# leok7v/sqz

Hardware: AMD Instinct MI355X
Metric: encode MB/s + decode MB/s, 32KB window, batched blocks, 1/2/4/8 MI355X (higher is better)
Workload: dtype u8; 1 GPU; 4096 x 262144 B Zipf(s=1) byte blocks, window 2^15, one independent stream per block (BASELINE.json configs[2]); total_blocks=4096, blocks_per_gpu=4096, block_bytes=262144, win_bits=15, parallelism=1 rank; the N>1 runs shard this same batch (strong scaling), finder=index, device=AMD Radeon Graphics (gfx950:sramecc+:xnack-)

## Files before the change

sqz_amd/csrc/decode.hip:

```cpp
#define SQZ_CHANGED_INLINING __forceinline__
#define SQZ_INSERT_INLINING __forceinline__
#define SQZ_LUT_INLINING __forceinline__
#include "sqz_tree.h"
#include "sqz_kernels.h"

namespace sqzk {

constexpr int kStageDw = 128;

struct DecodeLuts {
    uint16_t lit[1 << 8];
    uint16_t pos[1 << 6];
};

struct DecodeLds {
    TreeLds    tree;
    DecodeLuts luts;
    uint32_t   stage[kStageDw];
};

using LitTree = LitTreeT<false, false>;
using PosTree = PosTreeT<false, false>;

template <class T>
// ... 253 lines not shown
#endif
            ST_SEC(0)
            const int hop = ok ? (int)used : 128;
            uint64_t starts = 0;
            uint32_t s = 0;
            do {
                set_bit64(starts, s);
                s += (uint32_t)__builtin_amdgcn_readlane(hop, (int)s);
            } while (s < (uint32_t)kWave);
            if (s >= 128u) {
                stop = true;
                const int last = 63 - __builtin_clzll(starts);
                starts &= ~(1ull << last);
                s = (uint32_t)last;
            }
            base += s;
            if ((starts >> lane) & 1ull) {
                const int at = m + (int)__builtin_amdgcn_mbcnt_hi((uint32_t)(starts >> 32),
                                   __builtin_amdgcn_mbcnt_lo((uint32_t)starts, 0u));
                slot[at] = word | ((used - 1u) << 25);
            }
            m += __builtin_popcountll(starts);
            ST_SEC(1)
        }
        m = m < kWave ? m : kWave;
        ST_SEC(1)
        lds_fence();
        uint32_t word_v = 0, used_v = 0, slot_v = 0;
        if (lane < m) { slot_v = slot[lane]; word_v = slot_v & 0x81FFFFFFu; used_v = ((slot_v >> 25) & 63u) + 1u; }
        const bool is_match = (word_v & kTokMatch) != 0;
        const uint32_t tlen_v = lane < m ? (is_match ? ((word_v >> 16) & 0x1FFu) : 1u) : 0u;
        uint32_t scan = (used_v << 16) | tlen_v;
        scan = wave_scan(scan);
        const uint64_t out_before = i + (uint64_t)((scan & 0xFFFFu) - tlen_v);
        const bool invalid = lane < m &&
            (out_before >= bytes ||
             (is_match && ((uint64_t)(word_v & 0x7FFFu) > out_before + (kHist ? history : 0u) || (uint64_t)tlen_v > bytes - out_before)));
        const uint64_t inv = __ballot(invalid);
        if (inv != 0) { const int f = __builtin_ctzll(inv); if (f < m) { m = f; stop = true; } }
        int a_v = -1, b_v = -1;
        if (lane < m) {
            if (is_match) {
                a_v = kSymLen0 + len_code((int)tlen_v).code;
                b_v = kPosBase + pos_code((int)(word_v & 0x7FFFu)).code;
            } else {
                a_v = (int)word_v;
            }
        }
        uint32_t ca, cb;
        int wa, wb;
        int done = 0;
        ST_SEC(2)
        lds_fence();
        if (m > 0) { done = bump_batch<false>(&lds.tree, nullptr, lit, pos, lane, m, a_v, b_v, ca, wa, cb, wb); }
        ST_SEC(3)
        uint64_t resume = bit0;
        if (done > 0) {
            if (lane < done) { tok[ntok + (uint32_t)lane] = word_v; }
            const uint32_t af = (uint32_t)__builtin_amdgcn_readlane((int)scan, done - 1);
            ntok += (uint32_t)done;
            i += (uint64_t)(af & 0xFFFFu);
            resume = bit0 + (uint64_t)(af >> 16);
        }
#ifdef SQZ_STATS
        st_steps++; st_m += (uint32_t)m; st_done += (uint32_t)done;
#ifdef SQZ_STATS_SERIES
        if (lane == 0 && b == 1) { printf("S %d %d %d %d\n", want, m, done, (int)stop); }
#endif
        st_hist[done == 0 ? 0 : done < 8 ? 1 : done < 24 ? 2 : done < 64 ? 3 : 4]++;
#endif
        ST_SEC(4)
        if (i < bytes && (stop || done < m)) {
            const bool may_keep = done + 1 < m;
            if (may_keep && lane == 0) {
                lds.tree.pend[LitTree::kChgSlot] = 0x7FFFFFFFu; lds.tree.pend[LitTree::kChgSlot + 1] = 0u;
                lds.tree.pend[PosTree::kChgSlot] = 0x7FFFFFFFu; lds.tree.pend[PosTree::kChgSlot + 1] = 0u;
            }
            lds_fence();
            if (done < m) {
                const int sa = __builtin_amdgcn_readlane(a_v, done), sb = __builtin_amdgcn_readlane(b_v, done);
                const uint32_t w1 = (uint32_t)__builtin_amdgcn_readlane((int)word_v, done);
                const uint32_t u1 = (uint32_t)__builtin_amdgcn_readlane((int)used_v, done);
                const uint32_t l1 = (uint32_t)__builtin_amdgcn_readlane((int)tlen_v, done);
                { const Chain c = lit.chain_up(sa, lane); (void)lit.bump_wave(sa, c, lane); }
                if (sb >= 0) { const Chain c = pos.chain_up(sb, lane); (void)pos.bump_wave(sb, c, lane); }
                if (lit.fault | pos.fault) { err = kE2BIG; }
                else {
                    if (lane == 0) { tok[ntok] = w1; }
                    ntok++;
                    i += (uint64_t)l1;
                    r.seek(resume + (uint64_t)u1);
                }
            } else {
                r.seek(resume);
                decode_one();
            }
            lds_fence();
            const bool still = (lit.complete | pos.complete) == 0 && lit.depth < kFreezeDepth && pos.depth < kFreezeDepth &&
                               (lit.aux & pos.aux) != 0;
            if (may_keep && still && err == 0 && i < bytes) {
                const uint32_t la = lds.tree.pend[LitTree::kChgSlot], ha = lds.tree.pend[LitTree::kChgSlot + 1];
                const uint32_t lb = lds.tree.pend[PosTree::kChgSlot], hb = lds.tree.pend[PosTree::kChgSlot + 1];
                const bool cand = lane > done && lane < m;
                bool moved = false;
                if (cand) {
                    const uint32_t qa = r_pos(lds.tree.rng[a_v]);
                    moved = qa >= la && qa < ha;
// ... 382 lines not shown
                    if (fin >= (uint32_t)kWave) { stop = true; advance = (uint32_t)(kWave * v) + (fin - (uint32_t)kWave); }
                    else { entry = fin; advance = (uint32_t)(kWave * (v + 1)) + fin; }
                }
            }
            if (mine) {
                uint64_t starts = 0;
                uint32_t s1 = my_entry;
                while (s1 < (uint32_t)kWave) {
                    const uint32_t h = (uint32_t)__builtin_amdgcn_readlane(hop, (int)s1);
                    if (h >= 1024u) { break; }
                    set_bit64(starts, s1);
                    s1 += h;
                }
                if ((starts >> lane) & 1ull) { slot[my_base + (int)lanes_under(starts)] = word | ((used - 1u) << 25); }
            }
            base += advance;
            MW_SEC(3)
        }
        }
        MW_SEC(5)
        if (shared) { lds_barrier(); }
        if (wave != 0) { continue; }
        const int m_total = m;
        m = m < kWave ? m : kWave;
        lds_fence();
        uint32_t word_v = 0, used_v = 0, slot_v = 0;
        if (lane < m) { slot_v = slot[lane]; word_v = slot_v & 0x81FFFFFFu; used_v = ((slot_v >> 25) & 63u) + 1u; }
        const bool is_match = (word_v & kTokMatch) != 0;
        const uint32_t tlen_v = lane < m ? (is_match ? ((word_v >> 16) & 0x1FFu) : 1u) : 0u;
        uint32_t scan = (used_v << 16) | tlen_v;
        scan = wave_scan(scan);
        const uint64_t out_before = i + (uint64_t)((scan & 0xFFFFu) - tlen_v);
        const bool invalid = lane < m &&
            (out_before >= bytes ||
             (is_match && ((uint64_t)(word_v & 0x7FFFu) > out_before + (kHist ? history : 0u) || (uint64_t)tlen_v > bytes - out_before)));
        const uint64_t inv = __ballot(invalid);
        if (inv != 0) { const int f = __builtin_ctzll(inv); if (f < m) { m = f; stop = true; } }
        int a_v = -1, b_v = -1;
        if (lane < m) {
            if (is_match) {
                a_v = kSymLen0 + len_code((int)tlen_v).code;
                b_v = kPosBase + pos_code((int)(word_v & 0x7FFFu)).code;
            } else {
                a_v = (int)word_v;
            }
        }
        uint32_t ca, cb;
        int wa, wb;
        int done = 0;
        MW_SEC(6)
#ifdef SQZ_STATS
        mw_steps++;
#endif
        if (m > 0) { done = bump_batch<false>(&lds.tree, nullptr, lit, pos, lane, m, a_v, b_v, ca, wa, cb, wb); }
        MW_SEC(7)
#ifdef SQZ_STATS
        mw_done += (uint32_t)done;
#endif
        uint64_t resume = bit0;
        if (done > 0) {
            if (lane < done) { tok[ntok + (uint32_t)lane] = word_v; }
            const uint32_t af = (uint32_t)__builtin_amdgcn_readlane((int)scan, done - 1);
            ntok += (uint32_t)done;
            i += (uint64_t)(af & 0xFFFFu);
            resume = bit0 + (uint64_t)(af >> 16);
        }
        kept = 0; kept_bits = 0;
        int keep_from = done;
        if (i < bytes && (stop || done < m)) {
            const bool may_keep = done + 1 < m;
            if (may_keep && lane == 0) {
                lds.tree.pend[LitTree::kChgSlot] = 0x7FFFFFFFu; lds.tree.pend[LitTree::kChgSlot + 1] = 0u;
                lds.tree.pend[PosTree::kChgSlot] = 0x7FFFFFFFu; lds.tree.pend[PosTree::kChgSlot + 1] = 0u;
            }
            lds_fence();
            if (done < m) {
                const int sa = __builtin_amdgcn_readlane(a_v, done), sb = __builtin_amdgcn_readlane(b_v, done);
                const uint32_t w1 = (uint32_t)__builtin_amdgcn_readlane((int)word_v, done);
                const uint32_t u1 = (uint32_t)__builtin_amdgcn_readlane((int)used_v, done);
                const uint32_t l1 = (uint32_t)__builtin_amdgcn_readlane((int)tlen_v, done);
                { const Chain c = lit.chain_up(sa, lane); (void)lit.bump_wave(sa, c, lane); }
                if (sb >= 0) { const Chain c = pos.chain_up(sb, lane); (void)pos.bump_wave(sb, c, lane); }
                if (lit.fault | pos.fault) { err = kE2BIG; }
                else {
                    if (lane == 0) { tok[ntok] = w1; }
                    ntok++;
                    i += (uint64_t)l1;
                    r.seek(resume + (uint64_t)u1);
                }
            } else {
                r.seek(resume);
                decode_one();
            }
            lds_fence();
            const bool still = (lit.complete | pos.complete) == 0 && lit.depth < kFreezeDepth && pos.depth < kFreezeDepth &&
                               (lit.aux & pos.aux) != 0;
            if (may_keep && still && err == 0 && i < bytes) {
                const uint32_t la = lds.tree.pend[LitTree::kChgSlot], ha = lds.tree.pend[LitTree::kChgSlot + 1];
                const uint32_t lb = lds.tree.pend[PosTree::kChgSlot], hb = lds.tree.pend[PosTree::kChgSlot + 1];
                const bool cand = lane > done && lane < m;
                bool moved = false;
                if (cand) {
                    const uint32_t qa = r_pos(lds.tree.rng[a_v]);
                    moved = qa >= la && qa < ha;
                    if (is_match) { const uint32_t qb = r_pos(lds.tree.rng[b_v]); moved |= qb >= lb && qb < hb; }
                }
                const uint64_t behind = ~0ull << (done + 1);
// ... 220 lines not shown
```

sqz_amd/csrc/huffman_emit.hip:

```cpp
#define SQZ_SEC_TIMERS
#define SQZ_CHANGED_INLINING __forceinline__
#define SQZ_INSERT_INLINING __forceinline__
#include "sqz_tree.h"
#include "sqz_kernels.h"

namespace sqzk {

constexpr int kPendBits = 58;

struct EmitLds {
    TreeLds  tree;
    uint32_t code[kCodeSlots];
};


struct BitQueue {
    EmitLds* lds;
    uint8_t* out;
    uint64_t capacity;
    uint64_t bytes;
    uint64_t carry_v;
    int      carry;
    int      error;
    uint64_t pend_v;
    int      pend_n;

    __device__ __forceinline__ void store_words(int words, int lane) {
        if (error != 0 || words == 0) { return; }
        const uint64_t room = capacity - bytes;
        for (int k = lane; k < words; k += kWave) {
            const uint64_t w = lds->tree.P64[k];
            const uint64_t at = (uint64_t)k * 8;
            if (at + 8 <= room) {
                *reinterpret_cast<uint64_t*>(out + bytes + at) = __builtin_bswap64(w);
            } else {
                for (int j = 0; j < 8; j++) {
                    if (at + (uint64_t)j < room) { out[bytes + at + j] = (uint8_t)(w >> (56 - 8 * j)); }
                }
            }
        }
        if ((uint64_t)words * 8 <= room) { bytes += (uint64_t)words * 8; }
        else { bytes = capacity; error = kE2BIG; }
    }

    __device__ __forceinline__ void deposit(uint64_t v, uint32_t n, uint32_t o) {
        const uint32_t w = o >> 6, s = o & 63u;
        if (s + n <= 64) {
            atomicOr(reinterpret_cast<unsigned long long*>(&lds->tree.P64[w]),
                     (unsigned long long)v << (64 - s - n));
        } else {
            const uint32_t r = s + n - 64;
            atomicOr(reinterpret_cast<unsigned long long*>(&lds->tree.P64[w]),
                     (unsigned long long)(v >> r));
            atomicOr(reinterpret_cast<unsigned long long*>(&lds->tree.P64[w + 1]),
                     (unsigned long long)v << (64 - r));
        }
    }

    __device__ __forceinline__ void pack_lanes(uint64_t v1, uint32_t n1, uint64_t v2, uint32_t n2, int lane) {
        for (int k = lane; k < kImageWords; k += kWave) { lds->tree.P64[k] = (k == 0) ? carry_v : 0ull; }
        lds_fence();
        const uint32_t incl = wave_scan(n1 + n2);
        const uint32_t head = (uint32_t)carry + (uint32_t)pend_n;
        const uint32_t total = (uint32_t)__builtin_amdgcn_readlane((int)incl, kWave - 1) + head;
        if (pend_n != 0 && lane == 0) { deposit(pend_v, (uint32_t)pend_n, (uint32_t)carry); }
        const uint32_t at = head + incl - (n1 + n2);
        if (n1 != 0) { deposit(v1, n1, at); }
        if (n2 != 0) { deposit(v2, n2, at + n1); }
        lds_fence();
        const int words = (int)(total >> 6);
        store_words(words, lane);
        carry_v = uni64(lds->tree.P64[words]);
        lds_fence();
        carry = (int)(total & 63u);
        pend_v = 0; pend_n = 0;
    }

    __device__ __forceinline__ void pack(int lane) {
        if (pend_n != 0) { pack_lanes(0ull, 0u, 0ull, 0u, lane); }
    }

    __device__ __forceinline__ void push32(uint32_t value, int width, int lane) {
        if (pend_n + width > kPendBits) { pack(lane); }
        const uint64_t bits = width >= 32 ? (uint64_t)value : (uint64_t)(value & ((1u << width) - 1u));
        pend_v = (pend_v << width) | bits;
        pend_n += width;
    }
    __device__ __forceinline__ void push(uint64_t value, int width, int lane) {
        if (width > 32) {
            push32((uint32_t)(value >> 32), width - 32, lane);
            push32((uint32_t)value, 32, lane);
        } else {
            push32((uint32_t)value, width, lane);
        }
    }
    __device__ __forceinline__ void push_lsb(uint32_t value, int width, int lane) {
        push32(__brev(value) >> (32 - width), width, lane);
    }

    __device__ __forceinline__ void flush(int lane) {
        pack(lane);
        if (carry > 0) {
            if (lane == 0) { lds->tree.P64[0] = carry_v; }
            lds_fence();
            store_words(1, lane);
            carry = 0; carry_v = 0;
        }
    }
};

__device__ __noinline__ uint64_t deep_code(const uint32_t* lnk, int leaf, int& width) {
    uint64_t code = 0;
    int n = 0, a = leaf;
    for (;;) {
        const uint32_t up = (uint32_t)__builtin_amdgcn_readfirstlane((int)l_up(lnk[a]));
        if (up == kNil || n >= 63) { break; }
        const uint32_t pw = (uint32_t)__builtin_amdgcn_readfirstlane((int)lnk[up]);
        code |= (uint64_t)(l_hi(pw) == (uint32_t)a ? 1 : 0) << n;
        a = (int)up;
        n++;
    }
    width = n;
    return code;
}

template <class T>
__device__ __forceinline__ void emit_coded(BitQueue& q, T& t, int s, int nyt, int raw_bits,
                                           int lane, int& err) {
    Chain c = t.chain_up(s, lane);
    const bool unseen = (c.levels == 0);
    if (unseen) { c = t.chain_up(nyt, lane); }
    const int leaf = unseen ? nyt : s;
    int width = c.levels;
    uint64_t deep = 0;
    if (width >= kMaxFastDepth) { deep = deep_code(t.lds->lnk, leaf, width); }
    uint64_t code = t.bump_wave(leaf, c, lane);
    if (c.levels >= kMaxFastDepth) { code = deep; }
    q.push(code, width, lane);
    if (unseen) {
        q.push_lsb((uint32_t)(s - T::kBase), raw_bits, lane);
        if (!t.insert_wave(s, lane)) { err = kE2BIG; }
    }
}

template <class LitTree, class PosTree>
__device__ __forceinline__ void emit_token(BitQueue& q, LitTree& lit, PosTree& pos, uint32_t t,
                                           int lane, int& err) {
    const bool is_match = (t & kTokMatch) != 0;
    Code lc = {0, 0, 0};
    int s_lit = (int)(t & 0xFFu);
    if (is_match) {
        lc = len_code((int)((t >> 16) & 0x1FFu));
        s_lit = kSymLen0 + lc.code;
    }
    emit_coded(q, lit, s_lit, kLitNyt, 9, lane, err);
    if (is_match) {
        if (lc.xbits > 0) { q.push_lsb((uint32_t)lc.extra, lc.xbits, lane); }
        const Code pc = pos_code((int)(t & 0x7FFFu));
        emit_coded(q, pos, kPosBase + pc.code, kPosBase + kPosNyt, 5, lane, err);
        if (pc.xbits > 0) { q.push_lsb((uint32_t)pc.extra, pc.xbits, lane); }
    }
    if (q.error != 0) { err = q.error; }
    if (lit.fault | pos.fault) { err = kE2BIG; }
}

__device__ __forceinline__ bool token_ok(uint32_t t) {
    if ((t & kTokMatch) == 0) { return t <= 0xFFu; }
    const uint32_t len = (t >> 16) & 0x7FFFu, dist = t & 0xFFFFu;
    return len >= (uint32_t)kLenMin && len <= (uint32_t)kLenMax && dist >= 1u && dist <= 0x7FFFu;
}

template <bool kStats>
__global__ __launch_bounds__(kWave, kStats ? 1 : 4)
void huffman_emit_kernel(const uint32_t* __restrict__ tokens,
                         const uint64_t* __restrict__ tok_off,
                         const uint32_t* __restrict__ tok_count,
                         uint8_t* __restrict__ out,
                         const uint64_t* __restrict__ out_off,
                         uint64_t* __restrict__ out_bytes,
                         int32_t* __restrict__ err_out,
                         uint32_t n_blocks,
                         uint64_t prefix_acc, int prefix_fill,
                         sqz_block_stats* __restrict__ stats_out) {
    __shared__ EmitLds lds;
    const int lane = threadIdx.x;
    const uint32_t b = blockIdx.x;
    if (b >= n_blocks) { return; }

    using LitTree = LitTreeT<true, kStats>;
    using PosTree = PosTreeT<true, kStats>;
    LitTree lit; PosTree pos;
    lit.lds = &lds.tree; lit.code = lds.code; lit.lut = nullptr;
    pos.lds = &lds.tree; pos.code = lds.code; pos.lut = nullptr;
    lit.init_all(lane);
    pos.init_all(lane);
    for (int k = lane; k < kCodeSlots; k += kWave) { lds.code[k] = 0; }
    __syncthreads();

    const uint32_t* tok = tokens + uni64(tok_off[b]);
    uint32_t count = (uint32_t)__builtin_amdgcn_readfirstlane((int)tok_count[b]);
    const bool too_many = (uint64_t)count > uni64(tok_off[b + 1]) - uni64(tok_off[b]);
    if (too_many) { count = 0; }

    BitQueue q;
    q.lds = &lds;
    const uint64_t o0 = uni64(out_off[b]), o1 = uni64(out_off[b + 1]);
    q.out = out + o0;
    q.capacity = o1 - o0;
    q.bytes = 0;
    q.pend_v = 0;
    q.pend_n = 0;
    q.carry = prefix_fill;
    q.carry_v = prefix_fill > 0 ? (prefix_acc << (64 - prefix_fill)) : 0ull;
    q.error = 0;
    int err = 0;

    if (too_many) { err = kEINVAL; }
    if (!lit.insert_wave(kLitNyt, lane)) { err = kEINVAL; }
    if (!pos.insert_wave(kPosBase + kPosNyt, lane)) { err = kEINVAL; }

    uint32_t cursor = 0;
    uint32_t lit_tokens = 0, match_bytes = 0;
    uint32_t win0 = (uint32_t)lane < count ? tok[lane] : 0u;
    uint32_t win1 = (uint32_t)lane + (uint32_t)kWave < count ? tok[kWave + lane] : 0u;
#ifdef SQZ_STATS
    uint64_t es[4] = {0, 0, 0, 0}, es_last = __builtin_readcyclecounter(), es_begin = es_last;
    uint32_t es_steps = 0, es_exact = 0;
#define ES(k) { const uint64_t n_ = __builtin_readcyclecounter(); es[k] += n_ - es_last; es_last = n_; }
#else
#define ES(k)
#endif
    const uint32_t quarter = (count >> 2) + 1;
    int prio_now = -1;
    int want = 16, avg4 = 32;
    uint32_t regain_at = 0;
    while (cursor < count && err == 0) {
        {
            const int qq = (int)(cursor / quarter);
            if (qq != prio_now) {
                prio_now = qq;
                if (qq == 0) { __builtin_amdgcn_s_setprio(3); }
                else if (qq == 1) { __builtin_amdgcn_s_setprio(2); }
                else if (qq == 2) { __builtin_amdgcn_s_setprio(1); }
                else { __builtin_amdgcn_s_setprio(0); }
            }
        }
        const uint32_t step_start = cursor;
        const bool valid = cursor + (uint32_t)lane < count;
        const uint32_t traw = win0;
        const bool wellformed = token_ok(traw);
        const uint32_t t = wellformed ? traw : 0u;
        const bool is_match = (t & kTokMatch) != 0;
        Code lc = {0, 0, 0}, pc = {0, 0, 0};
        int a = (int)(t & 0xFFu), bsym = -1;
        uint32_t tlen = 1;
        if (is_match) {
            tlen = (t >> 16) & 0x1FFu;
            lc = len_code((int)tlen);
            pc = pos_code((int)(t & 0x7FFFu));
            a = kSymLen0 + lc.code;
            bsym = kPosBase + pc.code;
        }
        const bool new_a = valid && l_up(lds.tree.lnk[a]) == kNil;
        const bool new_b = valid && is_match && l_up(lds.tree.lnk[bsym]) == kNil;
        const uint64_t unseen = __ballot(valid && (new_a || new_b || !wellformed));
        const uint64_t vmask = __ballot(valid);
        int m = unseen != 0 ? __builtin_ctzll(unseen) : __builtin_popcountll(vmask);
        m = m < want ? m : want;
        if (cursor > kBatchTokens && (lit.aux | pos.aux) != 0) {
            lit.give_up_aux(lane);
            pos.give_up_aux(lane);
        }
        if ((lit.aux & pos.aux) == 0 && cursor <= kBatchTokens && cursor >= regain_at) {
            regain_at = cursor + 512u;
            (void)lit.regain_aux(lane);
            (void)pos.regain_aux(lane);
        }
        const bool frozen = (lit.complete | pos.complete) != 0 || lit.depth >= kFreezeDepth || pos.depth >= kFreezeDepth ||
                            (lit.aux & pos.aux) == 0;
        uint32_t ca = 0, cb = 0;
        int wa = 0, wb = 0;
        const int offered = m;
        ES(0)
        if (m >= 1 && !frozen) { m = bump_batch<true>(&lds.tree, lds.code, lit, pos, lane, m, a, bsym, ca, wa, cb, wb); }
        else { m = 0; }
        ES(1)
        if (m >= 1) {
            uint64_t v1 = ca, v2 = 0;
            uint32_t n1 = (uint32_t)wa, n2 = 0;
            if (is_match) {
                v1 = (v1 << lc.xbits) | (uint64_t)(lc.xbits ? (__brev((uint32_t)lc.extra) >> (32 - lc.xbits)) : 0u);
                n1 += (uint32_t)lc.xbits;
                v2 = ((uint64_t)cb << pc.xbits) | (uint64_t)(pc.xbits ? (__brev((uint32_t)pc.extra) >> (32 - pc.xbits)) : 0u);
                n2 = (uint32_t)(wb + pc.xbits);
            }
            if (lane >= m) { n1 = 0; n2 = 0; }
            q.pack_lanes(v1, n1, v2, n2, lane);
            if (kStats) {
                const uint64_t mm = __ballot(lane < m && is_match);
                lit_tokens += (uint32_t)(m - __builtin_popcountll(mm));
                match_bytes += wave_sum((lane < m && is_match) ? tlen : 0u);
            }
            cursor += (uint32_t)m;
        }
        ES(2)
        if (m < offered || offered == 0 || frozen) {
            const uint32_t tx = (uint32_t)__builtin_amdgcn_readlane((int)traw, m);
            if (!token_ok(tx)) { err = kEINVAL; break; }
            emit_token(q, lit, pos, tx, lane, err);
            if (kStats) { if ((tx & kTokMatch) != 0) { match_bytes += (tx >> 16) & 0x1FFu; } else { lit_tokens += 1; } }
            cursor += 1;
#ifdef SQZ_STATS
            es_exact++;
#endif
        }
        ES(3)
#ifdef SQZ_EMU_DEBUG_BATCH
        if (lane == 0) {
            static unsigned dbg_steps = 0, dbg_offered = 0, dbg_applied = 0, dbg_exact = 0, dbg_next = 16384;
            dbg_steps++; dbg_offered += (unsigned)offered - g_dbg_cut; g_dbg_cut = 0; dbg_applied += (unsigned)m; dbg_exact += (m < offered || offered == 0 || frozen) ? 1u : 0u;
            if (cursor >= dbg_next || cursor >= count) {
                fprintf(stderr, "cursor %u: steps %u offered %u applied %u exact %u (want %d) depth %d/%d aux %d/%d\n", cursor, dbg_steps, dbg_offered, dbg_applied, dbg_exact, want,
                        lit.depth, pos.depth, lit.aux, pos.aux);
                dbg_steps = dbg_offered = dbg_applied = dbg_exact = 0; dbg_next = cursor + 16384;
            }
        }
#endif
#ifdef SQZ_STATS
        es_steps++;
#endif
        {
            avg4 += (int)(cursor - step_start) - (avg4 >> 2);
            want = ((avg4 * 3) >> 3) + 6;
            want = want < kWave ? want : kWave;
        }
        {
            const uint32_t adv = cursor - step_start;
            const int from = ((lane + (int)adv) & (kWave - 1)) * 4;
            const uint32_t s0 = (uint32_t)__builtin_amdgcn_ds_bpermute(from, (int)win0);
            const uint32_t s1 = (uint32_t)__builtin_amdgcn_ds_bpermute(from, (int)win1);
            win0 = (uint32_t)lane + adv < (uint32_t)kWave ? s0 : s1;
            const uint32_t t1 = cursor + (uint32_t)kWave + (uint32_t)lane;
            win1 = t1 < count ? tok[t1] : 0u;
        }
        if (q.error != 0) { err = q.error; }
        if (lit.fault | pos.fault) { err = kE2BIG; }
    }

#ifdef SQZ_STATS
    if (lane == 0 && b == 1) {
        printf("emit block 1: cycles %llu steps %u exact %u: prep %llu bump %llu pack %llu exact %llu\n",
               (unsigned long long)(es_last - es_begin), es_steps, es_exact, (unsigned long long)es[0],
               (unsigned long long)es[1], (unsigned long long)es[2], (unsigned long long)es[3]);
        for (int k = 0; k < 32; k++) { if (g_secn[k]) { printf("sec %d: %llu cycles / %u = %llu\n", k, g_sec[k], g_secn[k], g_sec[k] / g_secn[k]); } }
        printf("emit slow: lit insert %u/%llu changed %u/%llu; pos insert %u/%llu changed %u/%llu\n",
               lit.st_cnt[0], (unsigned long long)lit.st_cyc[0], lit.st_cnt[1], (unsigned long long)lit.st_cyc[1],
               pos.st_cnt[0], (unsigned long long)pos.st_cyc[0], pos.st_cnt[1], (unsigned long long)pos.st_cyc[1]);
    }
#endif
    if (err == 0) { q.flush(lane); err = q.error; }
    else { q.pack(lane); }
    if (lane == 0) {
        out_bytes[b] = q.bytes;
        err_out[b] = err;
        if (kStats && stats_out != nullptr) {
            sqz_block_stats* st = stats_out + b;
            st->lit_updates = lit.stats.updates; st->lit_swaps = lit.stats.swaps; st->lit_moves = lit.stats.moves;
            st->pos_updates = pos.stats.updates; st->pos_swaps = pos.stats.swaps; st->pos_moves = pos.stats.moves;
            st->literal_bytes = lit_tokens; st->backref_bytes = match_bytes;
            st->lit_depth = (uint32_t)lit.depth; st->pos_depth = (uint32_t)pos.depth;
            st->tokens = cursor; st->reserved = 0;
        }
    }
    if (kStats && stats_out != nullptr) {
        for (int k = lane; k < kLitLeaves; k += kWave) { stats_out[b].lit_freq[k] = lit.freq(k); }
        if (lane < kPosLeaves) { stats_out[b].pos_freq[lane] = pos.freq(kPosBase + lane); }
    }
}

using DbgLit = LitTreeT<true, true>;
using DbgPos = PosTreeT<true, true>;
template <class T>
__device__ __forceinline__ void debug_drive(T& t, DbgLit& lit, DbgPos& pos, EmitLds& lds, const int32_t* symbols,
                                            uint32_t count, int batch, int lane, bool is_pos, bool stop_early,
                                            uint32_t max_steps, uint32_t& consumed) {
    uint32_t k = 0;
    for (uint32_t step = 0; k < count && t.fault == 0 && (max_steps == 0 || step < max_steps); step++) {
        if (stop_early && t.aux == 0) { break; }
        int sym = -1;
        if (k + (uint32_t)lane < count) { sym = symbols[k + lane]; }
        const bool valid = sym >= 0 && sym < T::kLeaves && lane < batch;
        const int leaf = valid ? T::kBase + sym : T::kRoot;
        const uint64_t seen = __ballot(valid && l_up(lds.tree.lnk[leaf]) != kNil);
        int m = (~seen == 0ull) ? kWave : __builtin_ctzll(~seen);
        const bool frozen = t.complete != 0 || t.depth >= kFreezeDepth || t.aux == 0;
        uint32_t ca, cb; int wa, wb;
        if (m > 0 && !frozen) {
            m = is_pos ? bump_batch<true>(&lds.tree, lds.code, lit, pos, lane, m, -1, leaf, ca, wa, cb, wb)
                       : bump_batch<true>(&lds.tree, lds.code, lit, pos, lane, m, leaf, -1, ca, wa, cb, wb);
        } else { m = 0; }
        k += (uint32_t)m;
        if (k < count) {
            const int s = __builtin_amdgcn_readfirstlane(symbols[k]);
            if (s < 0 || s >= T::kLeaves) { break; }
            const int lf = T::kBase + s;
            const Chain c = t.chain_up(lf, lane);
            if (c.levels == 0) { (void)t.insert_wave(lf, lane); }
            else { (void)t.bump_wave(lf, c, lane); }
            k++;
        }
    }
    consumed = k;
}

__global__ __launch_bounds__(kWave, 4)
void tree_debug_kernel(const int32_t* __restrict__ symbols, uint32_t count, int which, int batch,
                       uint32_t* __restrict__ dump) {
    __shared__ EmitLds lds;
    const int lane = threadIdx.x;
    DbgLit lit; DbgPos pos;
    lit.lds = &lds.tree; lit.code = lds.code; lit.lut = nullptr;
    pos.lds = &lds.tree; pos.code = lds.code; pos.lut = nullptr;
    lit.init_all(lane);
    pos.init_all(lane);
    for (int k = lane; k < kCodeSlots; k += kWave) { lds.code[k] = 0; }
    __syncthreads();
    const bool stop_early = (batch & 0x100) != 0;
    batch &= 0xFF;
    if (batch < 1) { batch = 1; }
    if (batch > kWave) { batch = kWave; }
    const uint32_t max_steps = (uint32_t)which >> 8;
    which &= 1;
    uint32_t consumed = 0;
    if (which == 0) { debug_drive(lit, lit, pos, lds, symbols, count, batch, lane, false, stop_early, max_steps, consumed); }
    else { debug_drive(pos, lit, pos, lds, symbols, count, batch, lane, true, stop_early, max_steps, consumed); }
    lds_fence();
    const int base = which == 0 ? 0 : kPosBase, nodes = which == 0 ? kLitNodes : kPosNodes;
    const int leaves = which == 0 ? kLitLeaves : kPosLeaves, pos0 = which == 0 ? 0 : kPosPos0;
    if (lane == 0) {
        const TreeStats st = which == 0 ? lit.stats : pos.stats;
        dump[0] = (uint32_t)(which == 0 ? lit.next : pos.next);
        dump[1] = (uint32_t)(which == 0 ? lit.depth : pos.depth);
        dump[2] = (uint32_t)(which == 0 ? lit.complete : pos.complete);
        dump[3] = (uint32_t)(which == 0 ? lit.aux : pos.aux);
        dump[4] = (uint32_t)(which == 0 ? lit.fault : pos.fault) | (max_steps != 0 ? consumed << 8 : 0u);
        dump[5] = st.updates; dump[6] = st.swaps; dump[7] = st.moves;
    }
    for (int v = lane; v < nodes; v += kWave) {
        dump[8 + 4 * v + 0] = lds.tree.lnk[base + v];
        dump[8 + 4 * v + 1] = lds.tree.rng[base + v];
        dump[8 + 4 * v + 2] = lds.tree.cnt[base + v];
        dump[8 + 4 * v + 3] = v < leaves ? lds.code[pos0 + v] : 0u;
// ... 28 lines not shown
```

sqz_amd/csrc/sqz_tree.h:

```cpp
#pragma once

#include "sqz_device.h"

namespace sqzk {

constexpr uint32_t kNil = 0x3FFu;
constexpr int kLitLeaves = 288;
constexpr int kLitNodes  = kLitLeaves + 288;
constexpr int kPosLeaves = 32;
constexpr int kPosNodes  = 64;
constexpr int kPosBase   = kLitNodes;
constexpr int kAllNodes  = kLitNodes + kPosNodes;
constexpr int kPosPos0   = kLitLeaves;
constexpr int kPositions = kLitLeaves + kPosLeaves;
constexpr int kCodeSlots = kPositions;

constexpr uint32_t kCountMask = (1u << 24) - 1u;
constexpr int kDepthShift = 24;

#ifndef SQZ_AUX_DEPTH
#define SQZ_AUX_DEPTH 26
#endif
#ifndef SQZ_MAX_FAST_DEPTH
#define SQZ_MAX_FAST_DEPTH 60
#endif
#ifndef SQZ_FREEZE_DEPTH
#define SQZ_FREEZE_DEPTH 63
#endif
#ifndef SQZ_BATCH_TOKENS
#define SQZ_BATCH_TOKENS ((1u << 24) - 256u)
#endif
constexpr uint32_t kBatchTokens = SQZ_BATCH_TOKENS;
constexpr int kAuxDepth = SQZ_AUX_DEPTH;
constexpr int kMaxFastDepth = SQZ_MAX_FAST_DEPTH;
constexpr int kFreezeDepth = SQZ_FREEZE_DEPTH;
constexpr int kStack = 128;
constexpr int kTokenBits = 2 * (kAuxDepth - 1) + 18;
constexpr int kPackWords = (63 + 58 + kWave * kTokenBits + 63) / 64 + 1;
constexpr int kImageWords = kPackWords > kWave ? kPackWords : kWave;

#ifdef SQZ_EMU_DEBUG_BATCH
static unsigned g_dbg_cut;
#endif

#if defined(SQZ_STATS) && defined(SQZ_SEC_TIMERS)
__device__ unsigned long long g_sec[32];
__device__ unsigned int g_secn[32];
#define SEC_BEGIN uint64_t sec_t_ = __builtin_readcyclecounter();
#define SEC(k) { const uint64_t n_ = __builtin_readcyclecounter(); if (blockIdx.x == 1 && threadIdx.x == 0) { g_sec[k] += n_ - sec_t_; g_secn[k]++; } sec_t_ = n_; }
#define XSEC_BEGIN uint64_t xsec_t_ = __builtin_readcyclecounter();
#define XSEC(k) { const uint64_t n_ = __builtin_readcyclecounter(); if (blockIdx.x == 1 && threadIdx.x == 0) { g_sec[k] += n_ - xsec_t_; g_secn[k]++; } xsec_t_ = n_; }
#else
#define SEC_BEGIN
#define SEC(k)
#define XSEC_BEGIN
#define XSEC(k)
#endif

struct TreeLds {
    uint32_t lnk[kAllNodes];
    uint32_t rng[kAllNodes];
    uint32_t cnt[kAllNodes];
    uint32_t pend[kWave];
    uint16_t lvl[kStack];
    union { uint64_t P64[kImageWords]; uint32_t P32[2 * kImageWords]; uint8_t P8[8 * kImageWords]; };
};

struct TreeStats { uint32_t updates, swaps, moves; };

__device__ __forceinline__ void lds_fence() {
    __builtin_amdgcn_fence(__ATOMIC_SEQ_CST, "wavefront");
    asm volatile("" ::: "memory");
}

__device__ __forceinline__ uint32_t l_up(uint32_t w) { return w & 0x3FFu; }
__device__ __forceinline__ uint32_t l_lo(uint32_t w) { return (w >> 10) & 0x3FFu; }
__device__ __forceinline__ uint32_t l_hi(uint32_t w) { return (w >> 20) & 0x3FFu; }
__device__ __forceinline__ uint32_t mk_lnk(uint32_t up, uint32_t lo, uint32_t hi) { return up | (lo << 10) | (hi << 20); }
__device__ __forceinline__ uint32_t r_pos(uint32_t w) { return w & 0x1FFu; }
__device__ __forceinline__ uint32_t r_first(uint32_t w) { return w & 0x3FFu; }
__device__ __forceinline__ uint32_t r_last(uint32_t w) { return (w >> 10) & 0x3FFu; }
__device__ __forceinline__ uint32_t r_pa(uint32_t w) { return (w >> 20) & 0x3FFu; }
constexpr uint32_t kEndsMask = 0xFFFFFu;
constexpr uint32_t kNoPos = 0x1FFu;
__device__ __forceinline__ uint32_t c_f(uint32_t w) { return w & kCountMask; }
__device__ __forceinline__ uint32_t c_d(uint32_t w) { return (w >> kDepthShift) & 0x3Fu; }

__device__ __forceinline__ uint32_t wave_max(uint32_t v) {
    auto mx = [](uint32_t a, uint32_t b) { return a > b ? a : b; };
    v = mx(v, (uint32_t)__builtin_amdgcn_update_dpp(0, (int)v, 0x111 , 0xf, 0xf, false));
    v = mx(v, (uint32_t)__builtin_amdgcn_update_dpp(0, (int)v, 0x112 , 0xf, 0xf, false));
    v = mx(v, (uint32_t)__builtin_amdgcn_update_dpp(0, (int)v, 0x114 , 0xf, 0xf, false));
    v = mx(v, (uint32_t)__builtin_amdgcn_update_dpp(0, (int)v, 0x118 , 0xf, 0xf, false));
    v = mx(v, (uint32_t)__builtin_amdgcn_update_dpp(0, (int)v, 0x142 , 0xa, 0xf, false));
    v = mx(v, (uint32_t)__builtin_amdgcn_update_dpp(0, (int)v, 0x143 , 0xc, 0xf, false));
    return (uint32_t)__builtin_amdgcn_readlane((int)v, kWave - 1);
}

__device__ __forceinline__ uint32_t wave_sum(uint32_t v) {
    return (uint32_t)__builtin_amdgcn_readlane((int)wave_scan(v), kWave - 1);
}

struct Chain {
    int mine, par;
    int levels;
    bool holds;
    bool active;
    bool has_g;
};

#ifndef SQZ_INSERT_INLINING
#define SQZ_INSERT_INLINING __noinline__
#endif
#ifndef SQZ_LUT_INLINING
#define SQZ_LUT_INLINING __noinline__
#endif
template <class T> __device__ SQZ_INSERT_INLINING uint32_t slow_insert(TreeLds* lds, uint32_t* code, uint32_t regs, int sym, int lane);
#ifndef SQZ_CHANGED_INLINING
#define SQZ_CHANGED_INLINING __noinline__
// ... 903 lines not shown
    if (t.depth + 4 >= kMaxFastDepth) {
        t.give_up_aux(lane);
        if (lane == 0) { t.changed(sym); }
        t.uniform_regs();
        lds_fence();
    } else {
        t.changed_all(t.make_chain(mine, levels, lane), lane);
    }
    t.store_stats_delta(lane);
    return (uint32_t)__builtin_amdgcn_readfirstlane((int)t.pack_regs());
}

template <class T>
__device__ __forceinline__ uint32_t lut_descend(const uint32_t* lnk, uint32_t parent, int bit, int level) {
    const uint32_t node = parent & 0x3FFu;
    const bool inside = node != kNil && node >= (uint32_t)T::kRoot;
    const uint32_t w = lnk[inside ? (int)node : (int)T::kRoot];
    const uint32_t child = bit ? l_hi(w) : l_lo(w);
    return inside ? (child | ((uint32_t)level << 10)) : parent;
}

template <class T>
__device__ SQZ_LUT_INLINING void slow_build_lut(const uint32_t* lnk, uint16_t* lut, int lane) {
    static_assert(T::kLutBits == 6 || T::kLutBits == 8, "table widths the decoder uses");
    const int half = (lane >> 1) * 4;
    const int bit = lane & 1;
    uint32_t e = (uint32_t)T::kRoot;
#pragma unroll
    for (int level = 1; level <= 6; level++) {
        const uint32_t parent = (uint32_t)__builtin_amdgcn_ds_bpermute(half, (int)e);
        e = lut_descend<T>(lnk, parent, bit, level);
    }
    if (T::kLutBits == 6) {
        lut[lane] = (uint16_t)e;
        return;
    }
    const uint32_t p0 = (uint32_t)__builtin_amdgcn_ds_bpermute(half, (int)e);
    const uint32_t p1 = (uint32_t)__builtin_amdgcn_ds_bpermute(half + 128, (int)e);
    const uint32_t r0 = lut_descend<T>(lnk, p0, bit, 7);
    const uint32_t r1 = lut_descend<T>(lnk, p1, bit, 7);
    const uint32_t q0 = (uint32_t)__builtin_amdgcn_ds_bpermute(half, (int)r0);
    const uint32_t q1 = (uint32_t)__builtin_amdgcn_ds_bpermute(half + 128, (int)r0);
    const uint32_t q2 = (uint32_t)__builtin_amdgcn_ds_bpermute(half, (int)r1);
    const uint32_t q3 = (uint32_t)__builtin_amdgcn_ds_bpermute(half + 128, (int)r1);
    lut[lane]       = (uint16_t)lut_descend<T>(lnk, q0, bit, 8);
    lut[lane + 64]  = (uint16_t)lut_descend<T>(lnk, q1, bit, 8);
    lut[lane + 128] = (uint16_t)lut_descend<T>(lnk, q2, bit, 8);
    lut[lane + 192] = (uint16_t)lut_descend<T>(lnk, q3, bit, 8);
}

template <bool CODES, bool STATS> using LitTreeT = Tree<0, kLitLeaves, kLitNodes, 512, 0, 8, CODES, STATS>;
template <bool CODES, bool STATS> using PosTreeT = Tree<kPosBase, kPosLeaves, kPosNodes, 32, kPosPos0, 6, CODES, STATS>;

template <bool kWantCode, class LIT, class POS>
__device__ __forceinline__ int bump_batch(TreeLds* lds, const uint32_t* code, const LIT& lit, const POS& pos,
                                          int lane, int m, int a, int b,
                                          uint32_t& code_a, int& depth_a, uint32_t& code_b, int& depth_b) {
    SEC_BEGIN
    const bool take = lane < m;
    bool has_a = take && a >= 0, has_b = take && b >= 0;
    const int ia = has_a ? a : LIT::kRoot - 1, ib = has_b ? b : POS::kRoot - 1;
    constexpr int kLitInner = kLitNodes - kLitLeaves, kPosInner = kPosNodes - kPosLeaves;
    constexpr int kLitRows = (kLitInner + kWave - 1) / kWave;
    constexpr int kLastRow = kLitRows - 1, kLastLit = kLastRow * kWave;
    static_assert(kLitInner % kWave != 0 && kLitInner % kWave <= kWave / 2, "the literal tree leaves half of its last row free");
    static_assert(kPosInner <= kWave / 2, "the distance tree's internal nodes fit that half row");
    static_assert(kPosPos0 >= kLitLeaves, "the leaf positions of the two trees do not overlap");
    int vi[kLitRows];
    bool on[kLitRows];
#pragma unroll
    for (int row = 0; row < kLastRow; row++) {
        const int v = LIT::kRoot + row * kWave + lane;
        on[row] = v < lit.next && v != LIT::kRoot;
        vi[row] = on[row] ? v : LIT::kRoot;
    }
    {
        const bool in_pos = lane >= kWave / 2;
        const int v = in_pos ? POS::kRoot + lane - kWave / 2 : LIT::kRoot + kLastLit + lane;
        on[kLastRow] = in_pos ? (v < pos.next && v != POS::kRoot) : v < lit.next;
        vi[kLastRow] = on[kLastRow] ? v : (in_pos ? POS::kRoot : LIT::kRoot);
    }
    const uint32_t ra = lds->rng[ia], rb = lds->rng[ib];
    const uint32_t wa = lds->cnt[ia], wb = lds->cnt[ib];
    uint32_t rw[kLitRows], cw[kLitRows];
#pragma unroll
    for (int k = 0; k < kLitRows; k++) { rw[k] = lds->rng[vi[k]]; cw[k] = lds->cnt[vi[k]]; }
    if (kWantCode) {
        code_a = code[has_a ? ia - LIT::kBase + 0 : 0];
        code_b = code[has_b ? ib - POS::kBase + kPosPos0 : 0];
    }
    const uint32_t qa = r_pos(ra), qb = r_pos(rb);
    depth_a = (int)c_d(wa);
    depth_b = (int)c_d(wb);
    const uint32_t pa_a = r_pa(ra), pa_b = r_pa(rb);
    const uint32_t cpa = lds->cnt[pa_a != kNil ? pa_a : (uint32_t)ia], cpb = lds->cnt[pa_b != kNil ? pa_b : (uint32_t)ib];
    uint32_t cp[kLitRows], rf[kLitRows], rl[kLitRows];
#pragma unroll
    for (int k = 0; k < kLitRows; k++) {
        const uint32_t pk = r_pa(rw[k]);
        cp[k] = lds->cnt[pk != kNil ? pk : (uint32_t)vi[k]];
        rf[k] = lds->rng[r_first(rw[k])];
        rl[k] = lds->rng[r_last(rw[k])];
    }
    SEC(0)
    auto clear_histogram = [&]() {
        lds->P64[lane] = 0ull;
        lds_fence();
    };
    auto histogram = [&](int upto) {
        if (lane < upto && has_a) { atomicAdd(&lds->P32[qa >> 2], 1u << (8u * (qa & 3u))); }
        if (lane < upto && has_b) { atomicAdd(&lds->P32[qb >> 2], 1u << (8u * (qb & 3u))); }
        lds_fence();
        const uint64_t h = lds->P64[lane];
        const uint64_t incl = h * 0x0101010101010101ull;
        const uint32_t total = (uint32_t)(incl >> 56);
        const uint32_t base = wave_scan(total) - total;
        lds->P64[lane] = (incl << 8) + (uint64_t)base * 0x0101010101010101ull;
        lds_fence();
    };
    clear_histogram();
#ifdef SQZ_EMU_DEBUG_BATCH
    const int dbg_m = m;
    const uint64_t dbg_sa = __ballot(has_a && pa_a != kNil && c_f(cpa) <= c_f(wa));
    const uint64_t dbg_sb = __ballot(has_b && pa_b != kNil && c_f(cpb) <= c_f(wb));
    const uint64_t dbg_nil = __ballot((has_a && pa_a == kNil) || (has_b && pa_b == kNil));
    uint64_t dbg_bad[2 + kLitRows] = {};
    auto dbg_line = [&](int cut, int applied) {
        if (lane != 0) { return; }
        fprintf(stderr, "batch m %d cut %d a %llx b %llx nil %llx bad", dbg_m, cut, (unsigned long long)dbg_sa,
                (unsigned long long)dbg_sb, (unsigned long long)dbg_nil);
        for (int c = 0; c < 2 + kLitRows; c++) { fprintf(stderr, " %llx", (unsigned long long)dbg_bad[c]); }
        fprintf(stderr, " ok %d next %d %d\n", applied, lit.next - LIT::kRoot, pos.next - POS::kRoot);
    };
#endif
#ifndef SQZ_BATCH_NO_CUT
    {
        const uint64_t stops = __ballot((has_a && pa_a != kNil && c_f(cpa) <= c_f(wa)) ||
                                        (has_b && pa_b != kNil && c_f(cpb) <= c_f(wb)));
        if (stops != 0) {
            const int j = __builtin_ctzll(stops);
#ifdef SQZ_EMU_DEBUG_BATCH
            if (lane == 0) { g_dbg_cut += (unsigned)(m - j); }
            if (j == 0) { dbg_line(0, 0); }
#endif
            m = j;
            if (m == 0) { return 0; }
            has_a = has_a && lane < m;
            has_b = has_b && lane < m;
        }
    }
#endif
    histogram(m);
    SEC(1)
    uint32_t st[kLitRows], en[kLitRows], pst[kLitRows], pen[kLitRows];
#pragma unroll
    for (int k = 0; k < kLitRows; k++) { st[k] = r_pos(rf[k]); en[k] = r_pos(rl[k]) + 1u; }
    const uint32_t p_a0 = lds->P8[qa], p_a1 = lds->P8[qa + 1u], p_b0 = lds->P8[qb], p_b1 = lds->P8[qb + 1u];
#pragma unroll
    for (int k = 0; k < kLitRows; k++) { pst[k] = lds->P8[st[k]]; pen[k] = lds->P8[en[k]]; }
    auto pack = [](uint32_t s0, uint32_t e0, uint32_t f, uint32_t fb) {
        const uint32_t allowed = fb > f ? fb - f : 0u;
        return s0 | (e0 << 9) | ((allowed < 255u ? allowed : 255u) << 18);
    };
    uint32_t nl[kLitRows], sel[kLitRows];
    uint32_t bad = 0;
    uint32_t sa, sb;
    {
        const uint32_t n = has_a ? p_a1 - p_a0 : 0u, f = c_f(wa), fb = c_f(cpa);
        sa = pack(qa, qa + 1u, f, fb);
        bad |= (n != 0 && pa_a != kNil && f + n > fb) ? 1u : 0u;
    }
    {
        const uint32_t n = has_b ? p_b1 - p_b0 : 0u, f = c_f(wb), fb = c_f(cpb);
        sb = pack(qb, qb + 1u, f, fb);
        bad |= (n != 0 && pa_b != kNil && f + n > fb) ? 2u : 0u;
    }
#pragma unroll
    for (int k = 0; k < kLitRows; k++) {
        const uint32_t n = on[k] ? pen[k] - pst[k] : 0u, f = c_f(cw[k]), fb = c_f(cp[k]);
        nl[k] = n;
        sel[k] = on[k] ? pack(st[k], en[k], f, fb) : 0u;
        bad |= (n != 0 && r_pa(rw[k]) != kNil && f + n > fb) ? (4u << k) : 0u;
    }
    int ok = m;
    SEC(2)
#ifdef SQZ_EMU_DEBUG_BATCH
    for (int c = 0; c < 2 + kLitRows; c++) { dbg_bad[c] = __ballot((bad >> c) & 1u); }
#endif
    if (__ballot(bad != 0) != 0) {
#pragma unroll
        for (int cat = 0; cat < 2 + kLitRows; cat++) {
            uint64_t vm = __ballot((bad >> cat) & 1u);
            const uint32_t mine = cat == 0 ? sa : cat == 1 ? sb : sel[cat >= 2 ? cat - 2 : 0];
            while (vm != 0) {
                const int k = __builtin_ctzll(vm);
                vm &= vm - 1;
                const uint32_t t = (uint32_t)__builtin_amdgcn_readlane((int)mine, k);
                const uint32_t s0 = t & 0x1FFu, e0 = (t >> 9) & 0x1FFu, allowed = t >> 18;
                const bool through = (has_a && qa >= s0 && qa < e0) || (has_b && qb >= s0 && qb < e0);
                const uint64_t tm = __ballot(through);
                const uint64_t first_bad = __ballot(through && lanes_under(tm) == allowed);
                if (first_bad != 0) { const int j = __builtin_ctzll(first_bad); ok = j < ok ? j : ok; }
            }
        }
#ifdef SQZ_EMU_DEBUG_BATCH
        if (ok == 0) { dbg_line(m < dbg_m ? m : -1, 0); }
#endif
        if (ok == 0) { return 0; }
        clear_histogram();
        histogram(ok);
#pragma unroll
        for (int row = 0; row < kLitRows; row++) {
            nl[row] = (uint32_t)lds->P8[(sel[row] >> 9) & 0x1FFu] - (uint32_t)lds->P8[sel[row] & 0x1FFu];
        }
    }
    SEC(3)
    if (lane < ok && has_a) { atomicAdd(&lds->cnt[ia], 1u); }
    if (lane < ok && has_b) { atomicAdd(&lds->cnt[ib], 1u); }
#pragma unroll
    for (int row = 0; row < kLitRows; row++) {
        if (nl[row] != 0) { atomicAdd(&lds->cnt[vi[row]], nl[row]); }
    }
    lds_fence();
    SEC(4)
#ifdef SQZ_EMU_DEBUG_BATCH
    dbg_line(m < dbg_m ? m : -1, ok);
#endif
    return ok;
}

}
```

Baseline: 15850 MB/s.

## Keep encoder bit image resident in LDS, drain only when full

The encoder's bit packer used to reset the LDS image, deposit bits and store whole words to global memory on every pack. It now accumulates into a persistent LDS image with a fill counter and drains to global only when the image would overflow, at capacity limits, or at flush. To stop the batched tree update from clobbering the image, the encoder's histogram moves into the adjacent pend/lvl LDS region through a new template flag. This cuts per-step clears, fences and small global stores, but the aliasing of pend/lvl relies on layout static_asserts and adds more drain logic.

```diff
diff --git a/sqz_amd/csrc/decode.hip b/sqz_amd/csrc/decode.hip
--- a/sqz_amd/csrc/decode.hip
+++ b/sqz_amd/csrc/decode.hip
@@ -329,7 +329,7 @@
         int done = 0;
         ST_SEC(2)
         lds_fence();
-        if (m > 0) { done = bump_batch<false>(&lds.tree, nullptr, lit, pos, lane, m, a_v, b_v, ca, wa, cb, wb); }
+        if (m > 0) { done = bump_batch<false, false>(&lds.tree, nullptr, lit, pos, lane, m, a_v, b_v, ca, wa, cb, wb); }
         ST_SEC(3)
         uint64_t resume = bit0;
         if (done > 0) {
@@ -818,7 +818,7 @@
 #ifdef SQZ_STATS
         mw_steps++;
 #endif
-        if (m > 0) { done = bump_batch<false>(&lds.tree, nullptr, lit, pos, lane, m, a_v, b_v, ca, wa, cb, wb); }
+        if (m > 0) { done = bump_batch<false, false>(&lds.tree, nullptr, lit, pos, lane, m, a_v, b_v, ca, wa, cb, wb); }
         MW_SEC(7)
 #ifdef SQZ_STATS
         mw_done += (uint32_t)done;
diff --git a/sqz_amd/csrc/huffman_emit.hip b/sqz_amd/csrc/huffman_emit.hip
--- a/sqz_amd/csrc/huffman_emit.hip
+++ b/sqz_amd/csrc/huffman_emit.hip
@@ -13,17 +13,38 @@
     uint32_t code[kCodeSlots];
 };
 
+constexpr uint32_t kImageBits = 64u * (uint32_t)kImageWords;
+static_assert(63 + kPendBits + kWave * kTokenBits < (int)kImageBits, "a step's bits fit the image after a drain");
+
+#ifdef SQZ_WAVE_EMU
+static unsigned g_dbg_drains, g_dbg_steps;
+#endif
+
+#if defined(SQZ_STATS) && defined(SQZ_SEC_TIMERS)
+#define PK_BEGIN uint64_t pk_t_ = __builtin_readcyclecounter();
+#define PK(k) { const uint64_t n_ = __builtin_readcyclecounter(); if (blockIdx.x == 1 && threadIdx.x == 0) { g_sec[k] += n_ - pk_t_; g_secn[k]++; } pk_t_ = n_; }
+#else
+#define PK_BEGIN
+#define PK(k)
+#endif
 
 struct BitQueue {
     EmitLds* lds;
     uint8_t* out;
     uint64_t capacity;
     uint64_t bytes;
-    uint64_t carry_v;
-    int      carry;
+    uint32_t fill;
     int      error;
     uint64_t pend_v;
     int      pend_n;
+
+    __device__ __forceinline__ void start(uint64_t prefix_acc, int prefix_fill, int lane) {
+        for (int k = lane; k < kImageWords; k += kWave) {
+            lds->tree.P64[k] = (k == 0 && prefix_fill > 0) ? (prefix_acc << (64 - prefix_fill)) : 0ull;
+        }
+        lds_fence();
+        fill = (uint32_t)prefix_fill;
+    }
 
     __device__ __forceinline__ void store_words(int words, int lane) {
         if (error != 0 || words == 0) { return; }
@@ -43,6 +64,26 @@
         else { bytes = capacity; error = kE2BIG; }
     }
 
+    __device__ __forceinline__ void drain(int lane) {
+        const int words = (int)(fill >> 6);
+        if (words == 0) { return; }
+#ifdef SQZ_WAVE_EMU
+        if (lane == 0) { g_dbg_drains++; }
+#endif
+        store_words(words, lane);
+        const uint64_t part = lds->tree.P64[words];
+        lds_fence();
+        for (int k = lane; k <= words; k += kWave) { lds->tree.P64[k] = (k == 0) ? part : 0ull; }
+        lds_fence();
+        fill &= 63u;
+    }
+
+    __device__ __forceinline__ void settle(uint32_t added, int lane) {
+        fill += added;
+        pend_v = 0; pend_n = 0;
+        if (error == 0 && (uint64_t)(fill >> 6) * 8 > capacity - bytes) { drain(lane); }
+    }
+
     __device__ __forceinline__ void deposit(uint64_t v, uint32_t n, uint32_t o) {
         const uint32_t w = o >> 6, s = o & 63u;
         if (s + n <= 64) {
@@ -58,26 +99,28 @@
     }
 
     __device__ __forceinline__ void pack_lanes(uint64_t v1, uint32_t n1, uint64_t v2, uint32_t n2, int lane) {
-        for (int k = lane; k < kImageWords; k += kWave) { lds->tree.P64[k] = (k == 0) ? carry_v : 0ull; }
-        lds_fence();
+        PK_BEGIN
         const uint32_t incl = wave_scan(n1 + n2);
-        const uint32_t head = (uint32_t)carry + (uint32_t)pend_n;
-        const uint32_t total = (uint32_t)__builtin_amdgcn_readlane((int)incl, kWave - 1) + head;
-        if (pend_n != 0 && lane == 0) { deposit(pend_v, (uint32_t)pend_n, (uint32_t)carry); }
-        const uint32_t at = head + incl - (n1 + n2);
+        const uint32_t added = (uint32_t)__builtin_amdgcn_readlane((int)incl, kWave - 1) + (uint32_t)pend_n;
+        PK(24)
+        if (fill + added >= kImageBits) { drain(lane); }
+        PK(26)
+        if (pend_n != 0 && lane == 0) { deposit(pend_v, (uint32_t)pend_n, fill); }
+        const uint32_t at = fill + (uint32_t)pend_n + incl - (n1 + n2);
         if (n1 != 0) { deposit(v1, n1, at); }
         if (n2 != 0) { deposit(v2, n2, at + n1); }
         lds_fence();
-        const int words = (int)(total >> 6);
-        store_words(words, lane);
-        carry_v = uni64(lds->tree.P64[words]);
+        PK(24)
+        settle(added, lane);
+        PK(26)
+    }
+
+    __device__ __forceinline__ void pack(int lane) {
+        if (pend_n == 0) { return; }
+        if (fill + (uint32_t)pend_n >= kImageBits) { drain(lane); }
+        if (lane == 0) { deposit(pend_v, (uint32_t)pend_n, fill); }
         lds_fence();
-        carry = (int)(total & 63u);
-        pend_v = 0; pend_n = 0;
-    }
-
-    __device__ __forceinline__ void pack(int lane) {
-        if (pend_n != 0) { pack_lanes(0ull, 0u, 0ull, 0u, lane); }
+        settle((uint32_t)pend_n, lane);
     }
 
     __device__ __forceinline__ void push32(uint32_t value, int width, int lane) {
@@ -100,12 +143,12 @@
 
     __device__ __forceinline__ void flush(int lane) {
         pack(lane);
-        if (carry > 0) {
-            if (lane == 0) { lds->tree.P64[0] = carry_v; }
-            lds_fence();
-            store_words(1, lane);
-            carry = 0; carry_v = 0;
-        }
+        drain(lane);
+        if (fill != 0) { fill = 64u; drain(lane); }
+    }
+    __device__ __forceinline__ void abandon(int lane) {
+        pack(lane);
+        drain(lane);
     }
 };
 
@@ -210,9 +253,8 @@
     q.bytes = 0;
     q.pend_v = 0;
     q.pend_n = 0;
-    q.carry = prefix_fill;
-    q.carry_v = prefix_fill > 0 ? (prefix_acc << (64 - prefix_fill)) : 0ull;
     q.error = 0;
+    q.start(prefix_acc, prefix_fill, lane);
     int err = 0;
 
     if (too_many) { err = kEINVAL; }
@@ -282,7 +324,7 @@
         int wa = 0, wb = 0;
         const int offered = m;
         ES(0)
-        if (m >= 1 && !frozen) { m = bump_batch<true>(&lds.tree, lds.code, lit, pos, lane, m, a, bsym, ca, wa, cb, wb); }
+        if (m >= 1 && !frozen) { m = bump_batch<true, true>(&lds.tree, lds.code, lit, pos, lane, m, a, bsym, ca, wa, cb, wb); }
         else { m = 0; }
         ES(1)
         if (m >= 1) {
@@ -329,6 +371,9 @@
 #ifdef SQZ_STATS
         es_steps++;
 #endif
+#ifdef SQZ_WAVE_EMU
+        if (lane == 0) { g_dbg_steps++; }
+#endif
         {
             avg4 += (int)(cursor - step_start) - (avg4 >> 2);
             want = ((avg4 * 3) >> 3) + 6;
@@ -359,7 +404,7 @@
     }
 #endif
     if (err == 0) { q.flush(lane); err = q.error; }
-    else { q.pack(lane); }
+    else { q.abandon(lane); }
     if (lane == 0) {
         out_bytes[b] = q.bytes;
         err_out[b] = err;
@@ -396,8 +441,8 @@
         const bool frozen = t.complete != 0 || t.depth >= kFreezeDepth || t.aux == 0;
         uint32_t ca, cb; int wa, wb;
         if (m > 0 && !frozen) {
-            m = is_pos ? bump_batch<true>(&lds.tree, lds.code, lit, pos, lane, m, -1, leaf, ca, wa, cb, wb)
-                       : bump_batch<true>(&lds.tree, lds.code, lit, pos, lane, m, leaf, -1, ca, wa, cb, wb);
+            m = is_pos ? bump_batch<true, true>(&lds.tree, lds.code, lit, pos, lane, m, -1, leaf, ca, wa, cb, wb)
+                       : bump_batch<true, true>(&lds.tree, lds.code, lit, pos, lane, m, leaf, -1, ca, wa, cb, wb);
         } else { m = 0; }
         k += (uint32_t)m;
         if (k < count) {
diff --git a/sqz_amd/csrc/sqz_tree.h b/sqz_amd/csrc/sqz_tree.h
--- a/sqz_amd/csrc/sqz_tree.h
+++ b/sqz_amd/csrc/sqz_tree.h
@@ -1,4 +1,6 @@
 #pragma once
+
+#include <cstddef>
 
 #include "sqz_device.h"
 
@@ -57,6 +59,9 @@
 #define XSEC(k)
 #endif
 
+typedef uint64_t __attribute__((may_alias)) hist_u64;
+typedef uint32_t __attribute__((may_alias)) hist_u32;
+
 struct TreeLds {
     uint32_t lnk[kAllNodes];
     uint32_t rng[kAllNodes];
@@ -64,7 +69,22 @@
     uint32_t pend[kWave];
     uint16_t lvl[kStack];
     union { uint64_t P64[kImageWords]; uint32_t P32[2 * kImageWords]; uint8_t P8[8 * kImageWords]; };
+
+    template <bool kInPend> __device__ __forceinline__ auto* hist64() {
+        if constexpr (kInPend) { return reinterpret_cast<hist_u64*>(pend); } else { return &P64[0]; }
+    }
+    template <bool kInPend> __device__ __forceinline__ auto* hist32() {
+        if constexpr (kInPend) { return reinterpret_cast<hist_u32*>(pend); } else { return &P32[0]; }
+    }
+    template <bool kInPend> __device__ __forceinline__ uint8_t* hist8() {
+        if constexpr (kInPend) { return reinterpret_cast<uint8_t*>(pend); } else { return &P8[0]; }
+    }
 };
+static_assert(offsetof(TreeLds, lvl) == offsetof(TreeLds, pend) + sizeof(uint32_t) * kWave, "pend and lvl are contiguous");
+static_assert(offsetof(TreeLds, pend) % 8 == 0, "the histogram's 64-bit words are aligned");
+static_assert(sizeof(uint32_t) * kWave + sizeof(uint16_t) * kStack >= 8 * (size_t)kWave, "clear_histogram writes one word per lane");
+static_assert(8 * kWave >= kPositions + 1, "a prefix sum per leaf position and one behind the last (41 words)");
+static_assert(offsetof(TreeLds, P64) == offsetof(TreeLds, pend) + 8 * (size_t)kWave, "the byte behind the encoder's histogram is the image's");
 
 struct TreeStats { uint32_t updates, swaps, moves; };
 
@@ -1074,7 +1094,7 @@
 template <bool CODES, bool STATS> using LitTreeT = Tree<0, kLitLeaves, kLitNodes, 512, 0, 8, CODES, STATS>;
 template <bool CODES, bool STATS> using PosTreeT = Tree<kPosBase, kPosLeaves, kPosNodes, 32, kPosPos0, 6, CODES, STATS>;
 
-template <bool kWantCode, class LIT, class POS>
+template <bool kWantCode, bool kHistInPend, class LIT, class POS>
 __device__ __forceinline__ int bump_batch(TreeLds* lds, const uint32_t* code, const LIT& lit, const POS& pos,
                                           int lane, int m, int a, int b,
                                           uint32_t& code_a, int& depth_a, uint32_t& code_b, int& depth_b) {
@@ -1125,19 +1145,22 @@
         rl[k] = lds->rng[r_last(rw[k])];
     }
     SEC(0)
+    auto* const H64 = lds->template hist64<kHistInPend>();
+    auto* const H32 = lds->template hist32<kHistInPend>();
+    const uint8_t* const H8 = lds->template hist8<kHistInPend>();
     auto clear_histogram = [&]() {
-        lds->P64[lane] = 0ull;
+        H64[lane] = 0ull;
         lds_fence();
     };
     auto histogram = [&](int upto) {
-        if (lane < upto && has_a) { atomicAdd(&lds->P32[qa >> 2], 1u << (8u * (qa & 3u))); }
-        if (lane < upto && has_b) { atomicAdd(&lds->P32[qb >> 2], 1u << (8u * (qb & 3u))); }
-        lds_fence();
-        const uint64_t h = lds->P64[lane];
+        if (lane < upto && has_a) { atomicAdd(&H32[qa >> 2], 1u << (8u * (qa & 3u))); }
+        if (lane < upto && has_b) { atomicAdd(&H32[qb >> 2], 1u << (8u * (qb & 3u))); }
+        lds_fence();
+        const uint64_t h = H64[lane];
         const uint64_t incl = h * 0x0101010101010101ull;
         const uint32_t total = (uint32_t)(incl >> 56);
         const uint32_t base = wave_scan(total) - total;
-        lds->P64[lane] = (incl << 8) + (uint64_t)base * 0x0101010101010101ull;
+        H64[lane] = (incl << 8) + (uint64_t)base * 0x0101010101010101ull;
         lds_fence();
     };
     clear_histogram();
@@ -1177,9 +1200,9 @@
     uint32_t st[kLitRows], en[kLitRows], pst[kLitRows], pen[kLitRows];
 #pragma unroll
     for (int k = 0; k < kLitRows; k++) { st[k] = r_pos(rf[k]); en[k] = r_pos(rl[k]) + 1u; }
-    const uint32_t p_a0 = lds->P8[qa], p_a1 = lds->P8[qa + 1u], p_b0 = lds->P8[qb], p_b1 = lds->P8[qb + 1u];
-#pragma unroll
-    for (int k = 0; k < kLitRows; k++) { pst[k] = lds->P8[st[k]]; pen[k] = lds->P8[en[k]]; }
+    const uint32_t p_a0 = H8[qa], p_a1 = H8[qa + 1u], p_b0 = H8[qb], p_b1 = H8[qb + 1u];
+#pragma unroll
+    for (int k = 0; k < kLitRows; k++) { pst[k] = H8[st[k]]; pen[k] = H8[en[k]]; }
     auto pack = [](uint32_t s0, uint32_t e0, uint32_t f, uint32_t fb) {
         const uint32_t allowed = fb > f ? fb - f : 0u;
         return s0 | (e0 << 9) | ((allowed < 255u ? allowed : 255u) << 18);
@@ -1233,7 +1256,7 @@
         histogram(ok);
 #pragma unroll
         for (int row = 0; row < kLitRows; row++) {
-            nl[row] = (uint32_t)lds->P8[(sel[row] >> 9) & 0x1FFu] - (uint32_t)lds->P8[sel[row] & 0x1FFu];
+            nl[row] = (uint32_t)H8[(sel[row] >> 9) & 0x1FFu] - (uint32_t)H8[sel[row] & 0x1FFu];
         }
     }
     SEC(3)
```

Measured after the change: 16190 MB/s, median of 6. 1.02x the previous value.
